# youssefg7/dl-sound-classification

Measured on AMD Instinct MI355X. Metric: training clips/sec (EnvNet-v2, ESC-50 shape), higher is better.
Workload: dtype bf16; 1 GPU; EnvNet-v2 train step (BC-mix, fwd, soft-CE, bwd, clip, Adam), ESC-50 shape; global_batch=256, per_gpu_batch=256, clip_samples=220500, parallelism=dp1, model=envnet_v2

## Files before the change

### dl-sound-classification_amd/csrc/pool.hip

```cpp
#include <cstdlib>

#include "channel_partials.h"

namespace {

constexpr int NT = CP_NT;

struct FastDiv {
  uint32_t d, m, l;
};
static FastDiv make_fastdiv(uint32_t d) {
  uint32_t l = 0;
  while ((1u << l) < d) ++l;
  const uint32_t m = (uint32_t)((((uint64_t)1 << 32) * (((uint64_t)1 << l) - d)) / d + 1);
  return FastDiv{d, m, l};
}
__device__ __forceinline__ uint32_t fdiv(uint32_t n, const FastDiv& f) { return (__umulhi(n, f.m) + n) >> f.l; }

__device__ __forceinline__ int64_t out_index(int layout, int b, int oy, int ox, int c, int OH, int OW, int C) {
  if (layout == 0) return (((int64_t)b * OH + oy) * OW + ox) * C + c;
  if (layout == 1) return ((int64_t)b * C + c) * OW + ox;
  return (((int64_t)b * C + c) * OH + oy) * OW + ox;
}

// ... 354 lines not shown
    }
    store8(dz, dtype, off, g);
  }
  cp_fold<2>(s1, s2, C, G, rslots, blockIdx.x, partial);
}

__global__ __launch_bounds__(NT) void pool_bwd_sparse_kernel(const void* __restrict__ dout, int layout,
                                                             const uint8_t* __restrict__ argmax,
                                                             const void* __restrict__ x,
                                                             const void* __restrict__ win, int dtype, int n, int H,
                                                             int W, int C, int kh, int kw,
                                                             const float* __restrict__ scale,
                                                             const float* __restrict__ shift,
                                                             const float* __restrict__ mean,
                                                             const float* __restrict__ invstd,
                                                             float* __restrict__ gm,
                                                             float* __restrict__ partial) {
  const int OH = H / kh, OW = W / kw, G = C / 8;
  const int t = threadIdx.x;
  const int cg = t % G, rs = t / G, rslots = NT / G;
  float sc[8], sh[8], mu[8], is[8];
#pragma unroll
  for (int i = 0; i < 8; ++i) {
    sc[i] = scale[cg * 8 + i]; sh[i] = shift[cg * 8 + i]; mu[i] = mean[cg * 8 + i]; is[i] = invstd[cg * 8 + i];
  }
  float s1[8] = {0}, s2[8] = {0};
  const int cells = n * OH * OW;
  for (int cell = blockIdx.x * rslots + rs; cell < cells; cell += gridDim.x * rslots) {
    const int ox = cell % OW;
    const int q = cell / OW;
    const int oy = q % OH;
// ... 11 lines not shown
        const uint32_t word = i < 4 ? am.x : am.y;
        const int a = (int)((word >> (8 * (i & 3))) & 0xffu);
        const int iy = oy * kh + a / kw, ix = ox * kw + a % kw;
        xv[i] = ld_elem(x, dtype, (((int64_t)b * H + iy) * W + ix) * C + cg * 8 + i);
        dv[i] = ld_elem(dout, dtype, out_index(layout, b, oy, ox, cg * 8 + i, OH, OW, C));
      }
    }
    float gv[8];
#pragma unroll
    for (int i = 0; i < 8; ++i) {
      const float g = fmaf(xv[i], sc[i], sh[i]) > 0.f ? dv[i] : 0.f;
      gv[i] = g;
      s1[i] += g;
      s2[i] = fmaf(g, (xv[i] - mu[i]) * is[i], s2[i]);
    }
    float4* gq = reinterpret_cast<float4*>(gm + (int64_t)cell * C + cg * 8);
    gq[0] = make_float4(gv[0], gv[1], gv[2], gv[3]);
    gq[1] = make_float4(gv[4], gv[5], gv[6], gv[7]);
  }
  __shared__ float red[NT * 16];
#pragma unroll
  for (int i = 0; i < 8; ++i) { red[t * 16 + i] = s1[i]; red[t * 16 + 8 + i] = s2[i]; }
  __syncthreads();
  for (int e = t; e < 2 * C; e += NT) {
    const int qq = e / C, c = e % C, g2 = c / 8, ci = c % 8;
    float acc = 0.f;
    for (int r2 = 0; r2 < rslots; ++r2) acc += red[(r2 * G + g2) * 16 + qq * 8 + ci];
    partial[((int64_t)blockIdx.x * C + c) * 2 + qq] = acc;
  }
}

__global__ __launch_bounds__(NT) void pool_bwd_sparse_tr_kernel(const void* __restrict__ dout,
                                                                const uint8_t* __restrict__ argmax,
                                                                const void* __restrict__ x,
                                                                const void* __restrict__ win, int dtype, int cells,
                                                                int H, int W, int C, int kh, int kw, int lg_nch,
                                                                const float* __restrict__ scale,
                                                                const float* __restrict__ shift,
                                                                const float* __restrict__ mean,
                                                                const float* __restrict__ invstd,
                                                                float* __restrict__ gm, float* __restrict__ partial) {
  const int OW = W / kw, S = (H / kh) * OW, G = C / 8;
  const int t = threadIdx.x;
  const int lb = xcd_block_id();
  const int cg = t % G, rs = t / G, rslots = NT / G;
  const int LD = C + 4;
  __shared__ __attribute__((aligned(16))) float red[NT * 16];
  float* tile = red;
  float sc[8], sh[8], mu[8], is[8];
#pragma unroll
  for (int i = 0; i < 8; ++i) {
    sc[i] = scale[cg * 8 + i]; sh[i] = shift[cg * 8 + i]; mu[i] = mean[cg * 8 + i]; is[i] = invstd[cg * 8 + i];
  }
  float s1[8] = {0}, s2[8] = {0};
  const int es = dtype == MIA_BF16 ? 1 : 2;
  const uintptr_t dbase = reinterpret_cast<uintptr_t>(dout) >> es;
// ... 51 lines not shown
        for (int i = 0; i < 8; ++i) {
          const uint32_t word = i < 4 ? am.x : am.y;
          const int a = (int)((word >> (8 * (i & 3))) & 0xffu);
          const int iy = oy * kh + a / kw, ix = ox * kw + a % kw;
          xv[i] = ld_elem(x, dtype, (((int64_t)b * H + iy) * W + ix) * C + cg * 8 + i);
        }
      }
      float gv[8];
#pragma unroll
      for (int i = 0; i < 8; ++i) {
        const float g = fmaf(xv[i], sc[i], sh[i]) > 0.f ? dv[i] : 0.f;
        gv[i] = g;
        s1[i] += g;
        s2[i] = fmaf(g, (xv[i] - mu[i]) * is[i], s2[i]);
      }
      float4* gq = reinterpret_cast<float4*>(gm + cell * C + cg * 8);
      gq[0] = make_float4(gv[0], gv[1], gv[2], gv[3]);
      gq[1] = make_float4(gv[4], gv[5], gv[6], gv[7]);
    }
    __syncthreads();
  }
  cp_fold<2>(s1, s2, C, G, rslots, lb, partial, red);
}

__global__ __launch_bounds__(NT) void pool_bn_bwd_apply_oct_kernel(const float* __restrict__ gm,
                                                                   const uint8_t* __restrict__ argmax,
                                                                   const bf16* __restrict__ x, int n, int H, int W,
                                                                   int C, int kh, int kw, FastDiv dNO, FastDiv dH,
                                                                   FastDiv dG, const float* __restrict__ gamma,
                                                                   const float* __restrict__ mean,
                                                                   const float* __restrict__ invstd,
                                                                   const float* __restrict__ dgamma,
                                                                   const float* __restrict__ dbeta, bf16* dx,
                                                                   float* __restrict__ partial) {
  const int OH = H / kh, OW = W / kw, G = C / 8, NO = (W + 7) / 8;
  const int t = threadIdx.x;
  const int cg = t % G;
  const int P = n * H * W;
  float mu[8], is[8], a[8], mb[8], mg[8];
  const float invP = 1.f / (float)P;
// ... 6 lines not shown
    mg[i] = dgamma[c] * invP;
  }
  float s1[8] = {0};
  const int64_t units = (int64_t)n * H * NO * G;
  for (int64_t u = (int64_t)blockIdx.x * NT + t; u < units; u += (int64_t)gridDim.x * NT) {
    const int rest = (int)fdiv((uint32_t)(u), dG);
    const int rowi = (int)fdiv((uint32_t)rest, dNO);
    const int o8 = rest - rowi * NO;
    const int iy = rowi - (int)fdiv((uint32_t)rowi, dH) * H;
    const int b = (rowi - iy) / H;
    const int ix0 = o8 * 8;
    const int oy = iy / kh, ox = ix0 / kw;
    const bool cell = oy < OH && ox < OW;
    const int64_t coff = cell ? (((int64_t)b * OH + oy) * OW + ox) * C + cg * 8 : 0;
    const uint2 am = *reinterpret_cast<const uint2*>(argmax + coff);
    const float4 g0 = reinterpret_cast<const float4*>(gm + coff)[0];
    const float4 g1 = reinterpret_cast<const float4*>(gm + coff)[1];
    const int64_t xoff = ((int64_t)rowi * W + ix0) * C + cg * 8;
    uint4 xr[8];
#pragma unroll
    for (int j = 0; j < 8; ++j) {
      const int64_t o = ix0 + j < W ? xoff + (int64_t)j * C : xoff;
      xr[j] = *reinterpret_cast<const uint4*>(x + o);
    }
    const float gv[8] = {g0.x, g0.y, g0.z, g0.w, g1.x, g1.y, g1.z, g1.w};
    const int pos0 = (iy - oy * kh) * kw + (ix0 - ox * kw);
#pragma unroll
    for (int j = 0; j < 8; ++j) {
      if (ix0 + j >= W) break;
      const uint32_t w4[4] = {xr[j].x, xr[j].y, xr[j].z, xr[j].w};
      uint32_t o4[4];
#pragma unroll
      for (int q = 0; q < 4; ++q) {
        float g[2];
#pragma unroll
        for (int h = 0; h < 2; ++h) {
          const int i = 2 * q + h;
          const float xv = __uint_as_float(h ? (w4[q] & 0xffff0000u) : (w4[q] << 16));
          const uint32_t word = i < 4 ? am.x : am.y;
          const int av = (int)((word >> (8 * (i & 3))) & 0xffu);
          const float gi = cell && av == pos0 + j ? gv[i] : 0.f;
          g[h] = a[i] * (gi - mb[i] - (xv - mu[i]) * is[i] * mg[i]);
          s1[i] += g[h];
        }
        o4[q] = pk_bf16(g[0], g[1]);
      }
      *reinterpret_cast<uint4*>(dx + xoff + (int64_t)j * C) = uint4{o4[0], o4[1], o4[2], o4[3]};
    }
  }
  if (partial) cp_fold<1>(s1, nullptr, C, G, NT / G, blockIdx.x, partial);
}

template <int KW, int RU>
__global__ __launch_bounds__(NT) void pool_bn_bwd_apply_run_kernel(const float* __restrict__ gm,
                                                                   const uint8_t* __restrict__ argmax,
                                                                   const bf16* __restrict__ x, int n, int H, int W,
                                                                   int C, int kh, FastDiv dNR, FastDiv dH, FastDiv dG,
                                                                   const float* __restrict__ gamma,
                                                                   const float* __restrict__ mean,
                                                                   const float* __restrict__ invstd,
                                                                   const float* __restrict__ dgamma,
                                                                   const float* __restrict__ dbeta, bf16* dx,
                                                                   float* __restrict__ partial) {
  const int OH = H / kh, OW = W / KW, G = C / 8, NR = (W + KW - 1) / KW;
  const int t = threadIdx.x;
  const int cg = t % G;
  const int P = n * H * W;
  float mu[8], is[8], a[8], mb[8], mg[8];
  const float invP = 1.f / (float)P;
#pragma unroll
  for (int i = 0; i < 8; ++i) {
    const int c = cg * 8 + i;
    mu[i] = mean[c]; is[i] = invstd[c];
    a[i] = (gamma ? gamma[c] : 1.f) * is[i];
    mb[i] = dbeta[c] * invP;
    mg[i] = dgamma[c] * invP;
  }
  float s1[8] = {0};
  const int units = n * H * NR * G;
  const int stride = gridDim.x * NT;
  for (int u0 = blockIdx.x * NT + t; u0 < units; u0 += RU * stride) {
    uint4 xr[RU][KW];
    uint2 am[RU];
    float4 g0[RU], g1[RU];
    int64_t xoff[RU];
    int pos0[RU], ix0[RU];
#pragma unroll
    for (int v = 0; v < RU; ++v) {
      const int u = min(u0 + v * stride, units - 1);
      const int rest = (int)fdiv((uint32_t)u, dG);
      const int rowi = (int)fdiv((uint32_t)rest, dNR);
      const int run = rest - rowi * NR;
      const int b = (int)fdiv((uint32_t)rowi, dH);
      const int iy = rowi - b * H;
      ix0[v] = run * KW;
      const int oy = iy / kh;
      const bool cell = oy < OH && run < OW;
      const int64_t coff = cell ? (((int64_t)b * OH + oy) * OW + run) * C + cg * 8 : 0;
      pos0[v] = cell ? (iy - oy * kh) * KW : -256;
      am[v] = *reinterpret_cast<const uint2*>(argmax + coff);
      g0[v] = reinterpret_cast<const float4*>(gm + coff)[0];
      g1[v] = reinterpret_cast<const float4*>(gm + coff)[1];
      xoff[v] = ((int64_t)rowi * W + ix0[v]) * C + cg * 8;
#pragma unroll
      for (int j = 0; j < KW; ++j) {
        const int64_t o = ix0[v] + j < W ? xoff[v] + (int64_t)j * C : xoff[v];
        xr[v][j] = *reinterpret_cast<const uint4*>(x + o);
      }
    }
#pragma unroll
    for (int v = 0; v < RU; ++v) {
      if (u0 + v * stride >= units) break;
      const float gv[8] = {g0[v].x, g0[v].y, g0[v].z, g0[v].w, g1[v].x, g1[v].y, g1[v].z, g1[v].w};
#pragma unroll
      for (int j = 0; j < KW; ++j) {
        if (ix0[v] + j >= W) break;
        const uint32_t w4[4] = {xr[v][j].x, xr[v][j].y, xr[v][j].z, xr[v][j].w};
        uint32_t o4[4];
#pragma unroll
        for (int q = 0; q < 4; ++q) {
          float g[2];
#pragma unroll
          for (int h = 0; h < 2; ++h) {
            const int i = 2 * q + h;
            const float xv = __uint_as_float(h ? (w4[q] & 0xffff0000u) : (w4[q] << 16));
            const uint32_t word = i < 4 ? am[v].x : am[v].y;
            const int av = (int)((word >> (8 * (i & 3))) & 0xffu);
            const float gi = av == pos0[v] + j ? gv[i] : 0.f;
// ... 6 lines not shown
      }
    }
  }
  if (partial) cp_fold<1>(s1, nullptr, C, G, NT / G, blockIdx.x, partial);
}

#ifndef PB_UNROLL
#define PB_UNROLL 4
#endif
#ifndef PB_NB
#define PB_NB CP_MAXBLK
#endif
#ifndef PB_RUNS
#define PB_RUNS 1
#endif
__global__ __launch_bounds__(NT) void pool_bn_bwd_apply_kernel(const float* __restrict__ gm,
                                                               const uint8_t* __restrict__ argmax,
                                                               const void* __restrict__ x, int dtype, int n, int H,
                                                               int W, int C, int kh, int kw, FastDiv dW, FastDiv dH,
                                                               FastDiv dkw, FastDiv dkh,
                                                               const float* __restrict__ gamma,
                                                               const float* __restrict__ mean,
                                                               const float* __restrict__ invstd,
                                                               const float* __restrict__ dgamma,
                                                               const float* __restrict__ dbeta, void* dx,
                                                               float* __restrict__ partial) {
  const int OH = H / kh, OW = W / kw, G = C / 8;
  const int t = threadIdx.x;
  const int cg = t % G, rs = t / G, rslots = NT / G;
  const int P = n * H * W;
  float mu[8], is[8], a[8], mb[8], mg[8];
  const float invP = 1.f / (float)P;
#pragma unroll
  for (int i = 0; i < 8; ++i) {
    const int c = cg * 8 + i;
    mu[i] = mean[c]; is[i] = invstd[c];
    a[i] = (gamma ? gamma[c] : 1.f) * is[i];
    mb[i] = dbeta[c] * invP;
    mg[i] = dgamma[c] * invP;
  }
  float s1[8] = {0};
  const int stride = gridDim.x * rslots;
  for (int r0 = blockIdx.x * rslots + rs; r0 < P; r0 += PB_UNROLL * stride) {
    float xv[PB_UNROLL][8];
    uint2 am[PB_UNROLL];
    float4 g0[PB_UNROLL], g1[PB_UNROLL];
#pragma unroll
    for (int u = 0; u < PB_UNROLL; ++u) {
      const int r = min(r0 + u * stride, P - 1);
      load8(x, dtype, (int64_t)r * C + cg * 8, xv[u]);
      const int q = (int)fdiv(r, dW), ix = r - q * W;
      const int b = (int)fdiv(q, dH), iy = q - b * H;
      const int oy = min((int)fdiv(iy, dkh), OH - 1), ox = min((int)fdiv(ix, dkw), OW - 1);
      const int64_t coff = (((int64_t)b * OH + oy) * OW + ox) * C + cg * 8;
      am[u] = *reinterpret_cast<const uint2*>(argmax + coff);
      g0[u] = reinterpret_cast<const float4*>(gm + coff)[0];
      g1[u] = reinterpret_cast<const float4*>(gm + coff)[1];
    }
#pragma unroll
    for (int u = 0; u < PB_UNROLL; ++u) {
      const int r = r0 + u * stride;
      if (r >= P) break;
      const int q = (int)fdiv(r, dW), ix = r - q * W;
      const int iy = q - (int)fdiv(q, dH) * H;
      const int oy = (int)fdiv(iy, dkh), ox = (int)fdiv(ix, dkw);
      const int pos = oy < OH && ox < OW ? (iy - oy * kh) * kw + (ix - ox * kw) : -1;
      const float gv[8] = {g0[u].x, g0[u].y, g0[u].z, g0[u].w, g1[u].x, g1[u].y, g1[u].z, g1[u].w};
      float g[8];
#pragma unroll
      for (int i = 0; i < 8; ++i) {
        const uint32_t word = i < 4 ? am[u].x : am[u].y;
        const int av = (int)((word >> (8 * (i & 3))) & 0xffu);
        const float gi = av == pos ? gv[i] : 0.f;
        g[i] = a[i] * (gi - mb[i] - (xv[u][i] - mu[i]) * is[i] * mg[i]);
        s1[i] += g[i];
      }
      store8(dx, dtype, (int64_t)r * C + cg * 8, g);
    }
  }
  if (partial) cp_fold<1>(s1, nullptr, C, G, rslots, blockIdx.x, partial);
}

// ... 94 lines not shown
  MIA_CHECK_ARG(c % 8 == 0 && c >= 8 && (NT % (c / 8)) == 0, "pool_bwd: channels");
  MIA_CHECK_ARG((int64_t)n * h * w < (1ll << 31), "pool_bwd: too many pixels for 32-bit indexing");
  const int rslots = NT / (c / 8);
  const int64_t P = (int64_t)n * h * w;
  hipStream_t s = as_stream(stream);
  const int nb = (int)std::max<int64_t>(1, std::min<int64_t>(cdiv(P, (int64_t)rslots * 8), CP_MAXBLK));
  pool_bwd_kernel<<<nb, NT, 0, s>>>(dout, out_layout, argmax, x, dtype, n, h, w, c, kh, kw, scale, shift, mean,
                                    invstd, dz, (float*)partial);
  MIA_LAUNCH_CHECK("pool_bwd");
  cp_final2_kernel<<<(unsigned)c, 256, 0, s>>>((const float*)partial, nb, c,  dbeta,
                                                dgamma);
  MIA_LAUNCH_CHECK("pool_bwd_final");
  return 0;
}

extern "C" int mia_pool_bwd_gather(const void* dout, int32_t out_layout, const uint8_t* argmax, const void* x,
                                   const void* win, int32_t dtype, int32_t n, int32_t h, int32_t w, int32_t c, int32_t kh, int32_t kw,
                                   const float* scale, const float* shift, const float* mean, const float* invstd,
                                   float* gm, float* dgamma, float* dbeta, void* partial, mia_stream_t stream) {
  MIA_CHECK_ARG(dout && argmax && x && scale && shift && mean && invstd && gm && dgamma && dbeta && partial,
                "pool_bwd_gather: null pointer");
  MIA_CHECK_ARG(c % 8 == 0 && c >= 8 && (NT % (c / 8)) == 0, "pool_bwd_gather: channels");
  MIA_CHECK_ARG((int64_t)n * h * w < (1ll << 31), "pool_bwd_gather: too many pixels for 32-bit indexing");
  MIA_CHECK_ARG(h >= kh && w >= kw && kh * kw <= 256 && (reinterpret_cast<uintptr_t>(gm) & 15) == 0,
                "pool_bwd_gather: bad geometry / alignment");
  const int rslots = NT / (c / 8);
  const int64_t cells = (int64_t)n * (h / kh) * (w / kw);
  const int nb = (int)std::max<int64_t>(1, std::min<int64_t>(cdiv(cells, (int64_t)rslots * 2), CP_MAXBLK));
  hipStream_t s = as_stream(stream);
  MIA_CHECK_ARG(!win || (reinterpret_cast<uintptr_t>(win) & 15) == 0, "pool_bwd_gather: win alignment");
  if (!pool_v1() && (out_layout == 2 || (out_layout == 1 && h / kh == 1)) && rslots >= 16 &&
      cells < (1ll << 31) - 1024) {
    int lg_nch = 0;
    while ((4 << lg_nch) < rslots) ++lg_nch;
    pool_bwd_sparse_tr_kernel<<<nb, NT, 0, s>>>(dout, argmax, x, win, dtype, (int)cells, h, w, c, kh, kw, lg_nch, scale,
                                                shift, mean, invstd, gm, (float*)partial);
  } else {
    pool_bwd_sparse_kernel<<<nb, NT, 0, s>>>(dout, out_layout, argmax, x, win, dtype, n, h, w, c, kh, kw, scale, shift,
                                             mean, invstd, gm, (float*)partial);
  }
  MIA_LAUNCH_CHECK("pool_bwd_gather");
  cp_final2_kernel<<<(unsigned)c, 256, 0, s>>>((const float*)partial, nb, c,  dbeta,
                                                dgamma);
  MIA_LAUNCH_CHECK("pool_bwd_gather_final");
  return 0;
}

extern "C" int mia_pool_bn_relu_bwd_apply(const float* gm, const uint8_t* argmax, const void* x, int32_t dtype,
                                          int32_t n, int32_t h, int32_t w, int32_t c, int32_t kh, int32_t kw,
                                          const float* gamma, const float* mean, const float* invstd,
                                          const float* dgamma, const float* dbeta, void* dx, float* dbias,
                                          void* partial, mia_stream_t stream) {
  MIA_CHECK_ARG(gm && argmax && x && mean && invstd && dgamma && dbeta && dx, "pool_bn_bwd_apply: null pointer");
  MIA_CHECK_ARG(!dbias || partial, "pool_bn_bwd_apply: dbias needs the partial workspace");
  MIA_CHECK_ARG(c % 8 == 0 && c >= 8 && (NT % (c / 8)) == 0, "pool_bn_bwd_apply: channels");
  MIA_CHECK_ARG((int64_t)n * h * w < (1ll << 31), "pool_bn_bwd_apply: too many pixels for 32-bit indexing");
  MIA_CHECK_ARG(h >= kh && w >= kw && kh * kw <= 256, "pool_bn_bwd_apply: bad geometry");
  const int rslots = NT / (c / 8);
  const int64_t P = (int64_t)n * h * w;
  hipStream_t s = as_stream(stream);
  const int64_t units = (int64_t)n * h * ((w + 7) / 8) * (c / 8);
  if (kw % 8 == 0 && dtype == MIA_BF16 && units < (1ll << 31) &&
      ((reinterpret_cast<uintptr_t>(x) | reinterpret_cast<uintptr_t>(dx)) & 15) == 0) {
    const int nb = (int)std::max<int64_t>(1, std::min<int64_t>(cdiv(units, NT), CP_MAXBLK));
    pool_bn_bwd_apply_oct_kernel<<<nb, NT, 0, s>>>(gm, argmax, reinterpret_cast<const bf16*>(x), n, h, w, c, kh, kw,
                                                   make_fastdiv((w + 7) / 8), make_fastdiv(h), make_fastdiv(c / 8),
                                                   gamma, mean, invstd, dgamma, dbeta, reinterpret_cast<bf16*>(dx),
                                                   dbias ? (float*)partial : nullptr);
    MIA_LAUNCH_CHECK("pool_bn_bwd_apply");
    if (dbias) {
      cp_final2_kernel<<<(unsigned)c, 256, 0, s>>>((const float*)partial, nb, c,  dbias, nullptr);
      MIA_LAUNCH_CHECK("pool_bn_bwd_apply_final");
    }
    return 0;
  }
  const int64_t runs = (int64_t)n * h * cdiv(w, kw) * (c / 8);
  static const bool per_pixel = getenv("MIA_POOL_BWD_PIXEL") != nullptr;
  if (kw >= 2 && kw <= 4 && dtype == MIA_BF16 && runs < (1ll << 31) && !per_pixel &&
      ((reinterpret_cast<uintptr_t>(x) | reinterpret_cast<uintptr_t>(dx)) & 15) == 0) {
    constexpr int RU = PB_RUNS;
    const int nb = (int)std::max<int64_t>(1, std::min<int64_t>(cdiv(runs, (int64_t)NT * RU), PB_NB));
    const FastDiv dNR = make_fastdiv((int)cdiv(w, kw)), dH = make_fastdiv(h), dG = make_fastdiv(c / 8);
    float* part = dbias ? (float*)partial : nullptr;
    const bf16* xb = reinterpret_cast<const bf16*>(x);
    bf16* dxb = reinterpret_cast<bf16*>(dx);
    if (kw == 2)
      pool_bn_bwd_apply_run_kernel<2, RU><<<nb, NT, 0, s>>>(gm, argmax, xb, n, h, w, c, kh, dNR, dH, dG, gamma, mean,
                                                            invstd, dgamma, dbeta, dxb, part);
    else if (kw == 3)
      pool_bn_bwd_apply_run_kernel<3, RU><<<nb, NT, 0, s>>>(gm, argmax, xb, n, h, w, c, kh, dNR, dH, dG, gamma, mean,
                                                            invstd, dgamma, dbeta, dxb, part);
    else
      pool_bn_bwd_apply_run_kernel<4, RU><<<nb, NT, 0, s>>>(gm, argmax, xb, n, h, w, c, kh, dNR, dH, dG, gamma, mean,
                                                            invstd, dgamma, dbeta, dxb, part);
    MIA_LAUNCH_CHECK("pool_bn_bwd_apply_run");
    if (dbias) {
      cp_final2_kernel<<<(unsigned)c, 256, 0, s>>>((const float*)partial, nb, c,  dbias, nullptr);
      MIA_LAUNCH_CHECK("pool_bn_bwd_apply_final");
    }
    return 0;
  }
  const int nb = (int)std::max<int64_t>(1, std::min<int64_t>(cdiv(P, (int64_t)rslots * 8), CP_MAXBLK));
  pool_bn_bwd_apply_kernel<<<nb, NT, 0, s>>>(gm, argmax, x, dtype, n, h, w, c, kh, kw, make_fastdiv(w), make_fastdiv(h),
                                             make_fastdiv(kw), make_fastdiv(kh), gamma, mean, invstd, dgamma,
                                             dbeta, dx, dbias ? (float*)partial : nullptr);
  MIA_LAUNCH_CHECK("pool_bn_bwd_apply");
  if (dbias) {
    cp_final2_kernel<<<(unsigned)c, 256, 0, s>>>((const float*)partial, nb, c,  dbias, nullptr);
    MIA_LAUNCH_CHECK("pool_bn_bwd_apply_final");
  }
  return 0;
}

extern "C" int mia_col2im_rows(const float* p, int32_t n, int32_t ph, int32_t w, int32_t kh, void* out, int32_t dtype,
                               mia_stream_t stream) {
  MIA_CHECK_ARG(p && out && n > 0 && ph > 0 && w > 0 && kh > 0, "col2im_rows: bad arguments");
  MIA_CHECK_ARG((int64_t)n * (ph + kh - 1) * w < (1ll << 31), "col2im_rows: too many elements");
  const int64_t total = (int64_t)n * (ph + kh - 1) * w;
  const int nb = (int)std::min<int64_t>(cdiv(total, 256), 16384);
  col2im_rows_kernel<<<nb, 256, 0, as_stream(stream)>>>(p, n, ph, w, kh, out, dtype);
  MIA_LAUNCH_CHECK("col2im_rows");
  return 0;
}
```

### dl-sound-classification_amd/src/miaudio/kernels.py

```python
from __future__ import annotations

import math
from dataclasses import dataclass

import os

import torch

from . import lib as L

_WS: dict = {}


def workspace(nbytes: int, device, slot: str = "main") -> torch.Tensor:
    key = (str(device), slot)
    buf = _WS.get(key)
    nbytes = max(int(nbytes), 256)
    if buf is None or buf.numel() < nbytes:
        buf = torch.empty(int(nbytes * 1.25) + 256, dtype=torch.uint8, device=device)
        _WS[key] = buf
    return buf


def _s():
# ... 285 lines not shown
    ws = workspace(lib.mia_bn_partial_bytes(P, C), x.device, "bn")
    L.check(lib.mia_bn_bwd_apply(dz.data_ptr(), x.data_ptr(), dx.data_ptr(), L.dtype_code(x), P, C,
                                 L.ptr(gamma), bn.mean.data_ptr(), bn.invstd.data_ptr(), dgamma.data_ptr(),
                                 dbeta.data_ptr(), L.ptr(dbias), ws.data_ptr(), _s()), "mia_bn_bwd_apply")


def bn_relu_bwd_apply(dact, x, dx, P, C, gamma, bn: BNState, dgamma, dbeta, dbias=None):
    lib = L.load()
    ws = workspace(lib.mia_bn_partial_bytes(P, C), x.device, "bn")
    L.check(lib.mia_bn_relu_bwd_apply(dact.data_ptr(), x.data_ptr(), dx.data_ptr(), L.dtype_code(x), P, C,
                                      L.ptr(gamma), bn.scale.data_ptr(), bn.shift.data_ptr(), bn.mean.data_ptr(),
                                      bn.invstd.data_ptr(), dgamma.data_ptr(), dbeta.data_ptr(), L.ptr(dbias),
                                      ws.data_ptr(), _s()), "mia_bn_relu_bwd_apply")


def pool_bwd_gather(dout, out_layout, argmax, x, n, h, w, c, kh, kw, bn: BNState, win=None):
    if win is not None and (win.dtype != x.dtype or win.numel() != n * (h // kh) * (w // kw) * c):
        raise ValueError("pool_bwd_gather: win must hold one x-typed value per pooled cell and channel")
    dev = x.device
    g = torch.empty(2, c, dtype=torch.float32, device=dev)
    gm = torch.empty(n * (h // kh) * (w // kw), c, dtype=torch.float32, device=dev)
    lib = L.load()
    ws = workspace(lib.mia_bn_partial_bytes(n * h * w, c), dev, "bn")
    L.check(lib.mia_pool_bwd_gather(dout.data_ptr(), out_layout, argmax.data_ptr(), x.data_ptr(), L.ptr(win),
                                    L.dtype_code(x), n, h, w, c, kh, kw, bn.scale.data_ptr(), bn.shift.data_ptr(), bn.mean.data_ptr(),
                                    bn.invstd.data_ptr(), gm.data_ptr(), g[0].data_ptr(), g[1].data_ptr(),
                                    ws.data_ptr(), _s()), "mia_pool_bwd_gather")
    return gm, g[0], g[1]


def pool_bn_relu_bwd_apply(gm, argmax, x, n, h, w, c, kh, kw, gamma, bn: BNState, dgamma, dbeta, dx, dbias=None):
    lib = L.load()
    ws = workspace(lib.mia_bn_partial_bytes(n * h * w, c), x.device, "bn")
    L.check(lib.mia_pool_bn_relu_bwd_apply(gm.data_ptr(), argmax.data_ptr(), x.data_ptr(), L.dtype_code(x), n, h, w,
                                           c, kh, kw, L.ptr(gamma), bn.mean.data_ptr(), bn.invstd.data_ptr(),
                                           dgamma.data_ptr(), dbeta.data_ptr(), dx.data_ptr(), L.ptr(dbias),
                                           ws.data_ptr(), _s()), "mia_pool_bn_relu_bwd_apply")


def pool_fwd(x, n, h, w, c, kh, kw, bn: BNState, out, out_layout, argmax, win=None):
    if win is not None and (win.dtype != x.dtype or win.numel() != n * (h // kh) * (w // kw) * c):
        raise ValueError("pool_fwd: win must hold one x-typed value per pooled cell and channel")
    L.check(L.load().mia_pool_fwd(x.data_ptr(), L.dtype_code(x), n, h, w, c, kh, kw, bn.scale.data_ptr(),
                                  bn.shift.data_ptr(), out.data_ptr(), out_layout, argmax.data_ptr(), L.ptr(win),
                                  _s()),
            "mia_pool_fwd")


def pool_raw_stats(x, n, h, w, c, kh, kw, gamma, kshift, win, argmax):
    assert x.dtype == torch.bfloat16 and win.dtype == torch.bfloat16 and x.is_contiguous()
    nblk = 2048
    part = torch.empty(nblk, c, 2, dtype=torch.float32, device=x.device)
# ... 759 lines not shown
```

### dl-sound-classification_amd/src/miaudio/lib.py

```python
from __future__ import annotations

import ctypes as C
import os
from pathlib import Path

import torch

PKG_ROOT = Path(__file__).resolve().parents[2]
LIB_PATH = Path(os.environ.get("MIAUDIO_LIB") or PKG_ROOT / "lib" / "libmiaudio.so")

F32, BF16, U8 = 0, 1, 2
MXFP8 = 16
OP_DENSE, OP_CONV, OP_CONVROW = 0, 1, 2
KC, RC = 0, 1
PRE_NONE, PRE_AFFINE, PRE_AFFINE_RELU, PRE_GELU = 0, 1, 2, 3
ACT_NONE, ACT_RELU, ACT_GELU, DACT_NZ, DACT_GELU, ACT_ADD_AUX, ACT_GELU_SAVE = 0, 1, 2, 3, 4, 5, 6
ACT_GELU_SAVE_D, DACT_MUL = 7, 8

vp = C.c_void_p
i32 = C.c_int32
i64 = C.c_int64
f32 = C.c_float


# ... 55 lines not shown
    "mia_gemm_mxfp8_ex": (C.c_int, [vp, vp, i64, vp, vp, i64, P(MiaEpilogue), i64, i64, i64, vp, vp]),
    "mia_layernorm_fwd_mx": (C.c_int, [vp, i32, vp, vp, vp, vp, vp, vp, vp, i64, i32, f32, vp]),
    "mia_attn_fwd_mx": (C.c_int, [vp, vp, vp, vp, vp, i32, i32, i32, f32, vp]),
    "mia_splitk_reduce": (C.c_int, [vp, i32, i64, i64, P(MiaEpilogue), vp]),
    "mia_logmel_workspace_bytes": (i64, [i64, i64]),
    "mia_logmel_fwd": (C.c_int, [vp, i64, i64, i64, P(MiaMelCfg), vp, vp, vp, vp, vp, vp, vp, vp, vp, vp, vp]),
    "mia_bn_partial_bytes": (i64, [i64, i32]),
    "mia_bn_fwd_stats": (C.c_int, [vp, i32, i64, i32, vp, vp, vp, vp, f32, f32, i32, vp, vp, vp, vp, vp, vp]),
    "mia_bn_relu_bwd_reduce": (C.c_int, [vp, vp, vp, i32, i64, i32, vp, vp, vp, vp, vp, vp, vp, vp]),
    "mia_bn_bwd_apply": (C.c_int, [vp, vp, vp, i32, i64, i32, vp, vp, vp, vp, vp, vp, vp, vp]),
    "mia_bn_relu_bwd_apply": (C.c_int, [vp, vp, vp, i32, i64, i32, vp, vp, vp, vp, vp, vp, vp, vp, vp, vp]),
    "mia_pool_bwd_gather": (C.c_int, [vp, i32, vp, vp, vp, i32, i32, i32, i32, i32, i32, i32, vp, vp, vp, vp, vp, vp,
                                      vp, vp, vp]),
    "mia_pool_bn_relu_bwd_apply": (C.c_int, [vp, vp, vp, i32, i32, i32, i32, i32, i32, i32, vp, vp, vp, vp, vp, vp,
                                             vp, vp, vp]),
    "mia_pool_fwd": (C.c_int, [vp, i32, i32, i32, i32, i32, i32, i32, vp, vp, vp, i32, vp, vp, vp]),
    "mia_pool_bwd_bn_relu_reduce": (C.c_int, [vp, i32, vp, vp, i32, i32, i32, i32, i32, i32, i32, vp, vp, vp,
                                              vp, vp, vp, vp, vp, vp]),
    "mia_colsum": (C.c_int, [vp, i32, i64, i32, i64, vp, vp, vp]),
    "mia_col2im_rows": (C.c_int, [vp, i32, i32, i32, i32, vp, i32, vp]),
    "mia_conv1ch_dgrad": (C.c_int, [vp, vp, vp, i32, i32, i32, vp]),
    "mia_fe_conv2_fwd": (C.c_int, [vp, vp, vp, vp, vp, vp, i32, i32, i32, vp]),
    "mia_fe_conv2_dgrad": (C.c_int, [vp, vp, vp, i32, i32, i32, vp]),
    "mia_bn_relu_apply": (C.c_int, [vp, i64, i32, vp, vp, vp, vp]),
    "mia_shift_pad_w2": (C.c_int, [vp, i64, i32, i32, vp, vp]),
    "mia_pad_w2": (C.c_int, [vp, i64, i32, i32, vp, vp, i32, vp]),
    "mia_drop_last_col": (C.c_int, [vp, i64, i32, i32, vp, vp]),
    "mia_fe_conv1_fwd": (C.c_int, [vp, vp, vp, vp, vp, i32, i32, i32, vp]),
    "mia_fe_conv3_fwd": (C.c_int, [vp, vp, vp, vp, vp, i32, i32, i32, i32, vp]),
    "mia_pool_raw_stats": (C.c_int, [vp, i32, i32, i32, i32, i32, i32, vp, vp, vp, vp, vp, i32, vp]),
# ... 152 lines not shown
```

Baseline: 15780 clips/s.

## Store pool backward gradient buffer in bf16 and add raw-window gather kernel

The intermediate pooled gradient buffer gm, passed between the pool backward gather and the BN-ReLU backward apply, now defaults to the activation dtype (bf16) instead of f32. This halves its write and read traffic. A new gather kernel for the row-major layout with a saved window reads win and dout as packed vectors directly, instead of decoding argmax and doing per-element gathers from x. The cost is extra gradient rounding to bf16 in the intermediate, which an env var can override back to f32.

```diff
diff --git a/dl-sound-classification_amd/csrc/pool.hip b/dl-sound-classification_amd/csrc/pool.hip
--- a/dl-sound-classification_amd/csrc/pool.hip
+++ b/dl-sound-classification_amd/csrc/pool.hip
@@ -1,5 +1,6 @@
 #include <cstdlib>
 
+#include "../../include/miaudio_pool.h"
 #include "channel_partials.h"
 
 namespace {
@@ -392,7 +393,7 @@
                                                              const float* __restrict__ shift,
                                                              const float* __restrict__ mean,
                                                              const float* __restrict__ invstd,
-                                                             float* __restrict__ gm,
+                                                             void* __restrict__ gm, int gdt,
                                                              float* __restrict__ partial) {
   const int OH = H / kh, OW = W / kw, G = C / 8;
   const int t = threadIdx.x;
@@ -434,9 +435,7 @@
       s1[i] += g;
       s2[i] = fmaf(g, (xv[i] - mu[i]) * is[i], s2[i]);
     }
-    float4* gq = reinterpret_cast<float4*>(gm + (int64_t)cell * C + cg * 8);
-    gq[0] = make_float4(gv[0], gv[1], gv[2], gv[3]);
-    gq[1] = make_float4(gv[4], gv[5], gv[6], gv[7]);
+    store8(gm, gdt, (int64_t)cell * C + cg * 8, gv);
   }
   __shared__ float red[NT * 16];
 #pragma unroll
@@ -448,6 +447,75 @@
     for (int r2 = 0; r2 < rslots; ++r2) acc += red[(r2 * G + g2) * 16 + qq * 8 + ci];
     partial[((int64_t)blockIdx.x * C + c) * 2 + qq] = acc;
   }
+}
+
+template <int DT>
+struct Raw8 {
+  uint4 v[DT == MIA_BF16 ? 1 : 2];
+  __device__ __forceinline__ void load(const void* p, int64_t off) {
+    const uint4* q = reinterpret_cast<const uint4*>(reinterpret_cast<const char*>(p) + off * (DT == MIA_BF16 ? 2 : 4));
+    v[0] = q[0];
+    if constexpr (DT != MIA_BF16) v[1] = q[1];
+  }
+  __device__ __forceinline__ void unpack(float (&f)[8]) const {
+    if constexpr (DT == MIA_BF16) {
+      const uint32_t w[4] = {v[0].x, v[0].y, v[0].z, v[0].w};
+#pragma unroll
+      for (int i = 0; i < 4; ++i) { f[2 * i] = __uint_as_float(w[i] << 16); f[2 * i + 1] = __uint_as_float(w[i] & 0xffff0000u); }
+    } else {
+      const uint32_t w[8] = {v[0].x, v[0].y, v[0].z, v[0].w, v[1].x, v[1].y, v[1].z, v[1].w};
+#pragma unroll
+      for (int i = 0; i < 8; ++i) f[i] = __uint_as_float(w[i]);
+    }
+  }
+};
+
+#ifndef PG_DEPTH
+#define PG_DEPTH 1
+#endif
+template <int DT, int GDT, int D>
+__global__ __launch_bounds__(NT) void pool_bwd_sparse_ra_kernel(const void* __restrict__ dout,
+                                                                const void* __restrict__ win, int cells, int C,
+                                                                const float* __restrict__ scale,
+                                                                const float* __restrict__ shift,
+                                                                const float* __restrict__ mean,
+                                                                const float* __restrict__ invstd,
+                                                                void* __restrict__ gm, float* __restrict__ partial) {
+  const int G = C / 8;
+  const int t = threadIdx.x;
+  const int cg = t % G, rs = t / G, rslots = NT / G;
+  float sc[8], sh[8], mu[8], is[8];
+#pragma unroll
+  for (int i = 0; i < 8; ++i) {
+    sc[i] = scale[cg * 8 + i]; sh[i] = shift[cg * 8 + i]; mu[i] = mean[cg * 8 + i]; is[i] = invstd[cg * 8 + i];
+  }
+  float s1[8] = {0}, s2[8] = {0};
+  const int stride = gridDim.x * rslots;
+  for (int cell0 = blockIdx.x * rslots + rs; cell0 < cells; cell0 += D * stride) {
+    Raw8<DT> wr[D], dr[D];
+#pragma unroll
+    for (int v = 0; v < D; ++v) {
+      const int64_t off = (int64_t)min(cell0 + v * stride, cells - 1) * C + cg * 8;
+      wr[v].load(win, off);
+      dr[v].load(dout, off);
+    }
+#pragma unroll
+    for (int v = 0; v < D; ++v) {
+      const bool live = cell0 + v * stride < cells;
+      float xv[8], dv[8], gv[8];
+      wr[v].unpack(xv);
+      dr[v].unpack(dv);
+#pragma unroll
+      for (int i = 0; i < 8; ++i) {
+        const float g = fmaf(xv[i], sc[i], sh[i]) > 0.f ? dv[i] : 0.f;
+        gv[i] = g;
+        s1[i] = live ? s1[i] + g : s1[i];
+        s2[i] = live ? fmaf(g, (xv[i] - mu[i]) * is[i], s2[i]) : s2[i];
+      }
+      if (live) store8(gm, GDT, (int64_t)(cell0 + v * stride) * C + cg * 8, gv);
+    }
+  }
+  cp_fold<2>(s1, s2, C, G, rslots, blockIdx.x, partial);
 }
 
 __global__ __launch_bounds__(NT) void pool_bwd_sparse_tr_kernel(const void* __restrict__ dout,
@@ -459,7 +527,8 @@
                                                                 const float* __restrict__ shift,
                                                                 const float* __restrict__ mean,
                                                                 const float* __restrict__ invstd,
-                                                                float* __restrict__ gm, float* __restrict__ partial) {
+                                                                void* __restrict__ gm, int gdt,
+                                                                float* __restrict__ partial) {
   const int OW = W / kw, S = (H / kh) * OW, G = C / 8;
   const int t = threadIdx.x;
   const int lb = xcd_block_id();
@@ -541,16 +610,15 @@
         s1[i] += g;
         s2[i] = fmaf(g, (xv[i] - mu[i]) * is[i], s2[i]);
       }
-      float4* gq = reinterpret_cast<float4*>(gm + cell * C + cg * 8);
-      gq[0] = make_float4(gv[0], gv[1], gv[2], gv[3]);
-      gq[1] = make_float4(gv[4], gv[5], gv[6], gv[7]);
+      store8(gm, gdt, cell * C + cg * 8, gv);
     }
     __syncthreads();
   }
   cp_fold<2>(s1, s2, C, G, rslots, lb, partial, red);
 }
 
-__global__ __launch_bounds__(NT) void pool_bn_bwd_apply_oct_kernel(const float* __restrict__ gm,
+template <int GDT>
+__global__ __launch_bounds__(NT) void pool_bn_bwd_apply_oct_kernel(const void* __restrict__ gm,
                                                                    const uint8_t* __restrict__ argmax,
                                                                    const bf16* __restrict__ x, int n, int H, int W,
                                                                    int C, int kh, int kw, FastDiv dNO, FastDiv dH,
@@ -587,8 +655,8 @@
     const bool cell = oy < OH && ox < OW;
     const int64_t coff = cell ? (((int64_t)b * OH + oy) * OW + ox) * C + cg * 8 : 0;
     const uint2 am = *reinterpret_cast<const uint2*>(argmax + coff);
-    const float4 g0 = reinterpret_cast<const float4*>(gm + coff)[0];
-    const float4 g1 = reinterpret_cast<const float4*>(gm + coff)[1];
+    Raw8<GDT> gr;
+    gr.load(gm, coff);
     const int64_t xoff = ((int64_t)rowi * W + ix0) * C + cg * 8;
     uint4 xr[8];
 #pragma unroll
@@ -596,7 +664,8 @@
       const int64_t o = ix0 + j < W ? xoff + (int64_t)j * C : xoff;
       xr[j] = *reinterpret_cast<const uint4*>(x + o);
     }
-    const float gv[8] = {g0.x, g0.y, g0.z, g0.w, g1.x, g1.y, g1.z, g1.w};
+    float gv[8];
+    gr.unpack(gv);
     const int pos0 = (iy - oy * kh) * kw + (ix0 - ox * kw);
 #pragma unroll
     for (int j = 0; j < 8; ++j) {
@@ -624,8 +693,8 @@
   if (partial) cp_fold<1>(s1, nullptr, C, G, NT / G, blockIdx.x, partial);
 }
 
-template <int KW, int RU>
-__global__ __launch_bounds__(NT) void pool_bn_bwd_apply_run_kernel(const float* __restrict__ gm,
+template <int KW, int RU, int GDT>
+__global__ __launch_bounds__(NT) void pool_bn_bwd_apply_run_kernel(const void* __restrict__ gm,
                                                                    const uint8_t* __restrict__ argmax,
                                                                    const bf16* __restrict__ x, int n, int H, int W,
                                                                    int C, int kh, FastDiv dNR, FastDiv dH, FastDiv dG,
@@ -655,7 +724,7 @@
   for (int u0 = blockIdx.x * NT + t; u0 < units; u0 += RU * stride) {
     uint4 xr[RU][KW];
     uint2 am[RU];
-    float4 g0[RU], g1[RU];
+    Raw8<GDT> gr[RU];
     int64_t xoff[RU];
     int pos0[RU], ix0[RU];
 #pragma unroll
@@ -672,8 +741,7 @@
       const int64_t coff = cell ? (((int64_t)b * OH + oy) * OW + run) * C + cg * 8 : 0;
       pos0[v] = cell ? (iy - oy * kh) * KW : -256;
       am[v] = *reinterpret_cast<const uint2*>(argmax + coff);
-      g0[v] = reinterpret_cast<const float4*>(gm + coff)[0];
-      g1[v] = reinterpret_cast<const float4*>(gm + coff)[1];
+      gr[v].load(gm, coff);
       xoff[v] = ((int64_t)rowi * W + ix0[v]) * C + cg * 8;
 #pragma unroll
       for (int j = 0; j < KW; ++j) {
@@ -684,7 +752,8 @@
 #pragma unroll
     for (int v = 0; v < RU; ++v) {
       if (u0 + v * stride >= units) break;
-      const float gv[8] = {g0[v].x, g0[v].y, g0[v].z, g0[v].w, g1[v].x, g1[v].y, g1[v].z, g1[v].w};
+      float gv[8];
+      gr[v].unpack(gv);
 #pragma unroll
       for (int j = 0; j < KW; ++j) {
         if (ix0[v] + j >= W) break;
@@ -721,7 +790,8 @@
 #ifndef PB_RUNS
 #define PB_RUNS 1
 #endif
-__global__ __launch_bounds__(NT) void pool_bn_bwd_apply_kernel(const float* __restrict__ gm,
+template <int GDT>
+__global__ __launch_bounds__(NT) void pool_bn_bwd_apply_kernel(const void* __restrict__ gm,
                                                                const uint8_t* __restrict__ argmax,
                                                                const void* __restrict__ x, int dtype, int n, int H,
                                                                int W, int C, int kh, int kw, FastDiv dW, FastDiv dH,
@@ -751,7 +821,7 @@
   for (int r0 = blockIdx.x * rslots + rs; r0 < P; r0 += PB_UNROLL * stride) {
     float xv[PB_UNROLL][8];
     uint2 am[PB_UNROLL];
-    float4 g0[PB_UNROLL], g1[PB_UNROLL];
+    Raw8<GDT> gr[PB_UNROLL];
 #pragma unroll
     for (int u = 0; u < PB_UNROLL; ++u) {
       const int r = min(r0 + u * stride, P - 1);
@@ -761,8 +831,7 @@
       const int oy = min((int)fdiv(iy, dkh), OH - 1), ox = min((int)fdiv(ix, dkw), OW - 1);
       const int64_t coff = (((int64_t)b * OH + oy) * OW + ox) * C + cg * 8;
       am[u] = *reinterpret_cast<const uint2*>(argmax + coff);
-      g0[u] = reinterpret_cast<const float4*>(gm + coff)[0];
-      g1[u] = reinterpret_cast<const float4*>(gm + coff)[1];
+      gr[u].load(gm, coff);
     }
 #pragma unroll
     for (int u = 0; u < PB_UNROLL; ++u) {
@@ -772,7 +841,8 @@
       const int iy = q - (int)fdiv(q, dH) * H;
       const int oy = (int)fdiv(iy, dkh), ox = (int)fdiv(ix, dkw);
       const int pos = oy < OH && ox < OW ? (iy - oy * kh) * kw + (ix - ox * kw) : -1;
-      const float gv[8] = {g0[u].x, g0[u].y, g0[u].z, g0[u].w, g1[u].x, g1[u].y, g1[u].z, g1[u].w};
+      float gv[8];
+      gr[u].unpack(gv);
       float g[8];
 #pragma unroll
       for (int i = 0; i < 8; ++i) {
@@ -897,30 +967,53 @@
   return 0;
 }
 
-extern "C" int mia_pool_bwd_gather(const void* dout, int32_t out_layout, const uint8_t* argmax, const void* x,
-                                   const void* win, int32_t dtype, int32_t n, int32_t h, int32_t w, int32_t c, int32_t kh, int32_t kw,
-                                   const float* scale, const float* shift, const float* mean, const float* invstd,
-                                   float* gm, float* dgamma, float* dbeta, void* partial, mia_stream_t stream) {
+static int pool_grid_cap(int nb) {
+  const char* e = getenv("MIA_POOL_GRID");
+  const int cap = e ? atoi(e) : 0;
+  return cap > 0 ? std::min(nb, cap) : nb;
+}
+
+extern "C" int mia_pool_bwd_gather_ex(const void* dout, int32_t out_layout, const uint8_t* argmax, const void* x,
+                                      const void* win, int32_t dtype, int32_t n, int32_t h, int32_t w, int32_t c,
+                                      int32_t kh, int32_t kw, const float* scale, const float* shift,
+                                      const float* mean, const float* invstd, void* gm, int32_t gm_dtype,
+                                      float* dgamma, float* dbeta, void* partial, mia_stream_t stream) {
   MIA_CHECK_ARG(dout && argmax && x && scale && shift && mean && invstd && gm && dgamma && dbeta && partial,
                 "pool_bwd_gather: null pointer");
   MIA_CHECK_ARG(c % 8 == 0 && c >= 8 && (NT % (c / 8)) == 0, "pool_bwd_gather: channels");
   MIA_CHECK_ARG((int64_t)n * h * w < (1ll << 31), "pool_bwd_gather: too many pixels for 32-bit indexing");
   MIA_CHECK_ARG(h >= kh && w >= kw && kh * kw <= 256 && (reinterpret_cast<uintptr_t>(gm) & 15) == 0,
                 "pool_bwd_gather: bad geometry / alignment");
+  MIA_CHECK_ARG(gm_dtype == MIA_F32 || (gm_dtype == MIA_BF16 && dtype == MIA_BF16),
+                "pool_bwd_gather: gm is f32, or bf16 beside bf16 activations (gm dtype %d, dtype %d)", gm_dtype, dtype);
   const int rslots = NT / (c / 8);
   const int64_t cells = (int64_t)n * (h / kh) * (w / kw);
-  const int nb = (int)std::max<int64_t>(1, std::min<int64_t>(cdiv(cells, (int64_t)rslots * 2), CP_MAXBLK));
+  const int nb = pool_grid_cap((int)std::max<int64_t>(1, std::min<int64_t>(cdiv(cells, (int64_t)rslots * 2), CP_MAXBLK)));
   hipStream_t s = as_stream(stream);
   MIA_CHECK_ARG(!win || (reinterpret_cast<uintptr_t>(win) & 15) == 0, "pool_bwd_gather: win alignment");
-  if (!pool_v1() && (out_layout == 2 || (out_layout == 1 && h / kh == 1)) && rslots >= 16 &&
-      cells < (1ll << 31) - 1024) {
+  const bool v1 = pool_v1();
+  const bool chmajor = out_layout == 2 || (out_layout == 1 && h / kh == 1);
+  if (!v1 && chmajor && rslots >= 16 && cells < (1ll << 31) - 1024) {
     int lg_nch = 0;
     while ((4 << lg_nch) < rslots) ++lg_nch;
     pool_bwd_sparse_tr_kernel<<<nb, NT, 0, s>>>(dout, argmax, x, win, dtype, (int)cells, h, w, c, kh, kw, lg_nch, scale,
-                                                shift, mean, invstd, gm, (float*)partial);
+                                                shift, mean, invstd, gm, gm_dtype, (float*)partial);
+  } else if (!v1 && win && out_layout == 0 && (dtype == MIA_BF16 || dtype == MIA_F32) &&
+             (reinterpret_cast<uintptr_t>(dout) & 15) == 0 && cells + (int64_t)PG_DEPTH * nb * rslots < (1ll << 31)) {
+    float* part = (float*)partial;
+    const int nc = (int)cells;
+    if (dtype == MIA_F32)
+      pool_bwd_sparse_ra_kernel<MIA_F32, MIA_F32, PG_DEPTH><<<nb, NT, 0, s>>>(dout, win, nc, c, scale, shift, mean,
+                                                                              invstd, gm, part);
+    else if (gm_dtype == MIA_F32)
+      pool_bwd_sparse_ra_kernel<MIA_BF16, MIA_F32, PG_DEPTH><<<nb, NT, 0, s>>>(dout, win, nc, c, scale, shift, mean,
+                                                                               invstd, gm, part);
+    else
+      pool_bwd_sparse_ra_kernel<MIA_BF16, MIA_BF16, PG_DEPTH><<<nb, NT, 0, s>>>(dout, win, nc, c, scale, shift, mean,
+                                                                                invstd, gm, part);
   } else {
     pool_bwd_sparse_kernel<<<nb, NT, 0, s>>>(dout, out_layout, argmax, x, win, dtype, n, h, w, c, kh, kw, scale, shift,
-                                             mean, invstd, gm, (float*)partial);
+                                             mean, invstd, gm, gm_dtype, (float*)partial);
   }
   MIA_LAUNCH_CHECK("pool_bwd_gather");
   cp_final2_kernel<<<(unsigned)c, 256, 0, s>>>((const float*)partial, nb, c,  dbeta,
@@ -929,27 +1022,29 @@
   return 0;
 }
 
-extern "C" int mia_pool_bn_relu_bwd_apply(const float* gm, const uint8_t* argmax, const void* x, int32_t dtype,
-                                          int32_t n, int32_t h, int32_t w, int32_t c, int32_t kh, int32_t kw,
-                                          const float* gamma, const float* mean, const float* invstd,
-                                          const float* dgamma, const float* dbeta, void* dx, float* dbias,
-                                          void* partial, mia_stream_t stream) {
-  MIA_CHECK_ARG(gm && argmax && x && mean && invstd && dgamma && dbeta && dx, "pool_bn_bwd_apply: null pointer");
-  MIA_CHECK_ARG(!dbias || partial, "pool_bn_bwd_apply: dbias needs the partial workspace");
-  MIA_CHECK_ARG(c % 8 == 0 && c >= 8 && (NT % (c / 8)) == 0, "pool_bn_bwd_apply: channels");
-  MIA_CHECK_ARG((int64_t)n * h * w < (1ll << 31), "pool_bn_bwd_apply: too many pixels for 32-bit indexing");
-  MIA_CHECK_ARG(h >= kh && w >= kw && kh * kw <= 256, "pool_bn_bwd_apply: bad geometry");
+extern "C" int mia_pool_bwd_gather(const void* dout, int32_t out_layout, const uint8_t* argmax, const void* x,
+                                   const void* win, int32_t dtype, int32_t n, int32_t h, int32_t w, int32_t c, int32_t kh, int32_t kw,
+                                   const float* scale, const float* shift, const float* mean, const float* invstd,
+                                   float* gm, float* dgamma, float* dbeta, void* partial, mia_stream_t stream) {
+  return mia_pool_bwd_gather_ex(dout, out_layout, argmax, x, win, dtype, n, h, w, c, kh, kw, scale, shift, mean, invstd,
+                                gm, MIA_F32, dgamma, dbeta, partial, stream);
+}
+
+template <int GDT>
+static int pool_bn_bwd_apply_launch(const void* gm, const uint8_t* argmax, const void* x, int32_t dtype, int32_t n,
+                                    int32_t h, int32_t w, int32_t c, int32_t kh, int32_t kw, const float* gamma,
+                                    const float* mean, const float* invstd, const float* dgamma, const float* dbeta,
+                                    void* dx, float* dbias, void* partial, hipStream_t s) {
   const int rslots = NT / (c / 8);
   const int64_t P = (int64_t)n * h * w;
-  hipStream_t s = as_stream(stream);
   const int64_t units = (int64_t)n * h * ((w + 7) / 8) * (c / 8);
   if (kw % 8 == 0 && dtype == MIA_BF16 && units < (1ll << 31) &&
       ((reinterpret_cast<uintptr_t>(x) | reinterpret_cast<uintptr_t>(dx)) & 15) == 0) {
     const int nb = (int)std::max<int64_t>(1, std::min<int64_t>(cdiv(units, NT), CP_MAXBLK));
-    pool_bn_bwd_apply_oct_kernel<<<nb, NT, 0, s>>>(gm, argmax, reinterpret_cast<const bf16*>(x), n, h, w, c, kh, kw,
-                                                   make_fastdiv((w + 7) / 8), make_fastdiv(h), make_fastdiv(c / 8),
-                                                   gamma, mean, invstd, dgamma, dbeta, reinterpret_cast<bf16*>(dx),
-                                                   dbias ? (float*)partial : nullptr);
+    pool_bn_bwd_apply_oct_kernel<GDT><<<nb, NT, 0, s>>>(gm, argmax, reinterpret_cast<const bf16*>(x), n, h, w, c, kh, kw,
+                                                        make_fastdiv((w + 7) / 8), make_fastdiv(h), make_fastdiv(c / 8),
+                                                        gamma, mean, invstd, dgamma, dbeta, reinterpret_cast<bf16*>(dx),
+                                                        dbias ? (float*)partial : nullptr);
     MIA_LAUNCH_CHECK("pool_bn_bwd_apply");
     if (dbias) {
       cp_final2_kernel<<<(unsigned)c, 256, 0, s>>>((const float*)partial, nb, c,  dbias, nullptr);
@@ -968,14 +1063,14 @@
     const bf16* xb = reinterpret_cast<const bf16*>(x);
     bf16* dxb = reinterpret_cast<bf16*>(dx);
     if (kw == 2)
-      pool_bn_bwd_apply_run_kernel<2, RU><<<nb, NT, 0, s>>>(gm, argmax, xb, n, h, w, c, kh, dNR, dH, dG, gamma, mean,
-                                                            invstd, dgamma, dbeta, dxb, part);
+      pool_bn_bwd_apply_run_kernel<2, RU, GDT><<<nb, NT, 0, s>>>(gm, argmax, xb, n, h, w, c, kh, dNR, dH, dG, gamma,
+                                                                 mean, invstd, dgamma, dbeta, dxb, part);
     else if (kw == 3)
-      pool_bn_bwd_apply_run_kernel<3, RU><<<nb, NT, 0, s>>>(gm, argmax, xb, n, h, w, c, kh, dNR, dH, dG, gamma, mean,
-                                                            invstd, dgamma, dbeta, dxb, part);
+      pool_bn_bwd_apply_run_kernel<3, RU, GDT><<<nb, NT, 0, s>>>(gm, argmax, xb, n, h, w, c, kh, dNR, dH, dG, gamma,
+                                                                 mean, invstd, dgamma, dbeta, dxb, part);
     else
-      pool_bn_bwd_apply_run_kernel<4, RU><<<nb, NT, 0, s>>>(gm, argmax, xb, n, h, w, c, kh, dNR, dH, dG, gamma, mean,
-                                                            invstd, dgamma, dbeta, dxb, part);
+      pool_bn_bwd_apply_run_kernel<4, RU, GDT><<<nb, NT, 0, s>>>(gm, argmax, xb, n, h, w, c, kh, dNR, dH, dG, gamma,
+                                                                 mean, invstd, dgamma, dbeta, dxb, part);
     MIA_LAUNCH_CHECK("pool_bn_bwd_apply_run");
     if (dbias) {
       cp_final2_kernel<<<(unsigned)c, 256, 0, s>>>((const float*)partial, nb, c,  dbias, nullptr);
@@ -984,15 +1079,44 @@
     return 0;
   }
   const int nb = (int)std::max<int64_t>(1, std::min<int64_t>(cdiv(P, (int64_t)rslots * 8), CP_MAXBLK));
-  pool_bn_bwd_apply_kernel<<<nb, NT, 0, s>>>(gm, argmax, x, dtype, n, h, w, c, kh, kw, make_fastdiv(w), make_fastdiv(h),
-                                             make_fastdiv(kw), make_fastdiv(kh), gamma, mean, invstd, dgamma,
-                                             dbeta, dx, dbias ? (float*)partial : nullptr);
+  pool_bn_bwd_apply_kernel<GDT><<<nb, NT, 0, s>>>(gm, argmax, x, dtype, n, h, w, c, kh, kw, make_fastdiv(w),
+                                                  make_fastdiv(h), make_fastdiv(kw), make_fastdiv(kh), gamma, mean,
+                                                  invstd, dgamma, dbeta, dx, dbias ? (float*)partial : nullptr);
   MIA_LAUNCH_CHECK("pool_bn_bwd_apply");
   if (dbias) {
     cp_final2_kernel<<<(unsigned)c, 256, 0, s>>>((const float*)partial, nb, c,  dbias, nullptr);
     MIA_LAUNCH_CHECK("pool_bn_bwd_apply_final");
   }
   return 0;
+}
+
+extern "C" int mia_pool_bn_relu_bwd_apply_ex(const void* gm, int32_t gm_dtype, const uint8_t* argmax, const void* x,
+                                             int32_t dtype, int32_t n, int32_t h, int32_t w, int32_t c, int32_t kh,
+                                             int32_t kw, const float* gamma, const float* mean, const float* invstd,
+                                             const float* dgamma, const float* dbeta, void* dx, float* dbias,
+                                             void* partial, mia_stream_t stream) {
+  MIA_CHECK_ARG(gm && argmax && x && mean && invstd && dgamma && dbeta && dx, "pool_bn_bwd_apply: null pointer");
+  MIA_CHECK_ARG(!dbias || partial, "pool_bn_bwd_apply: dbias needs the partial workspace");
+  MIA_CHECK_ARG(c % 8 == 0 && c >= 8 && (NT % (c / 8)) == 0, "pool_bn_bwd_apply: channels");
+  MIA_CHECK_ARG((int64_t)n * h * w < (1ll << 31), "pool_bn_bwd_apply: too many pixels for 32-bit indexing");
+  MIA_CHECK_ARG(h >= kh && w >= kw && kh * kw <= 256, "pool_bn_bwd_apply: bad geometry");
+  MIA_CHECK_ARG(gm_dtype == MIA_F32 || gm_dtype == MIA_BF16, "pool_bn_bwd_apply: gm dtype %d", gm_dtype);
+  MIA_CHECK_ARG((reinterpret_cast<uintptr_t>(gm) & 15) == 0, "pool_bn_bwd_apply: gm alignment");
+  hipStream_t s = as_stream(stream);
+  if (gm_dtype == MIA_BF16)
+    return pool_bn_bwd_apply_launch<MIA_BF16>(gm, argmax, x, dtype, n, h, w, c, kh, kw, gamma, mean, invstd, dgamma,
+                                              dbeta, dx, dbias, partial, s);
+  return pool_bn_bwd_apply_launch<MIA_F32>(gm, argmax, x, dtype, n, h, w, c, kh, kw, gamma, mean, invstd, dgamma, dbeta,
+                                           dx, dbias, partial, s);
+}
+
+extern "C" int mia_pool_bn_relu_bwd_apply(const float* gm, const uint8_t* argmax, const void* x, int32_t dtype,
+                                          int32_t n, int32_t h, int32_t w, int32_t c, int32_t kh, int32_t kw,
+                                          const float* gamma, const float* mean, const float* invstd,
+                                          const float* dgamma, const float* dbeta, void* dx, float* dbias,
+                                          void* partial, mia_stream_t stream) {
+  return mia_pool_bn_relu_bwd_apply_ex(gm, MIA_F32, argmax, x, dtype, n, h, w, c, kh, kw, gamma, mean, invstd, dgamma,
+                                       dbeta, dx, dbias, partial, stream);
 }
 
 extern "C" int mia_col2im_rows(const float* p, int32_t n, int32_t ph, int32_t w, int32_t kh, void* out, int32_t dtype,
diff --git a/dl-sound-classification_amd/src/miaudio/kernels.py b/dl-sound-classification_amd/src/miaudio/kernels.py
--- a/dl-sound-classification_amd/src/miaudio/kernels.py
+++ b/dl-sound-classification_amd/src/miaudio/kernels.py
@@ -323,28 +323,32 @@
                                       ws.data_ptr(), _s()), "mia_bn_relu_bwd_apply")
 
 
-def pool_bwd_gather(dout, out_layout, argmax, x, n, h, w, c, kh, kw, bn: BNState, win=None):
+def pool_bwd_gather(dout, out_layout, argmax, x, n, h, w, c, kh, kw, bn: BNState, win=None, gm_dtype=None):
     if win is not None and (win.dtype != x.dtype or win.numel() != n * (h // kh) * (w // kw) * c):
         raise ValueError("pool_bwd_gather: win must hold one x-typed value per pooled cell and channel")
+    if gm_dtype is None:
+        gm_dtype = torch.float32 if os.environ.get("MIA_POOL_GM32", "")[:1] == "1" else x.dtype
     dev = x.device
     g = torch.empty(2, c, dtype=torch.float32, device=dev)
-    gm = torch.empty(n * (h // kh) * (w // kw), c, dtype=torch.float32, device=dev)
+    gm = torch.empty(n * (h // kh) * (w // kw), c, dtype=gm_dtype, device=dev)
     lib = L.load()
     ws = workspace(lib.mia_bn_partial_bytes(n * h * w, c), dev, "bn")
-    L.check(lib.mia_pool_bwd_gather(dout.data_ptr(), out_layout, argmax.data_ptr(), x.data_ptr(), L.ptr(win),
-                                    L.dtype_code(x), n, h, w, c, kh, kw, bn.scale.data_ptr(), bn.shift.data_ptr(), bn.mean.data_ptr(),
-                                    bn.invstd.data_ptr(), gm.data_ptr(), g[0].data_ptr(), g[1].data_ptr(),
-                                    ws.data_ptr(), _s()), "mia_pool_bwd_gather")
+    L.check(lib.mia_pool_bwd_gather_ex(dout.data_ptr(), out_layout, argmax.data_ptr(), x.data_ptr(), L.ptr(win),
+                                       L.dtype_code(x), n, h, w, c, kh, kw, bn.scale.data_ptr(), bn.shift.data_ptr(),
+                                       bn.mean.data_ptr(), bn.invstd.data_ptr(), gm.data_ptr(), L.dtype_code(gm),
+                                       g[0].data_ptr(), g[1].data_ptr(), ws.data_ptr(), _s()),
+            "mia_pool_bwd_gather_ex")
     return gm, g[0], g[1]
 
 
 def pool_bn_relu_bwd_apply(gm, argmax, x, n, h, w, c, kh, kw, gamma, bn: BNState, dgamma, dbeta, dx, dbias=None):
     lib = L.load()
     ws = workspace(lib.mia_bn_partial_bytes(n * h * w, c), x.device, "bn")
-    L.check(lib.mia_pool_bn_relu_bwd_apply(gm.data_ptr(), argmax.data_ptr(), x.data_ptr(), L.dtype_code(x), n, h, w,
-                                           c, kh, kw, L.ptr(gamma), bn.mean.data_ptr(), bn.invstd.data_ptr(),
-                                           dgamma.data_ptr(), dbeta.data_ptr(), dx.data_ptr(), L.ptr(dbias),
-                                           ws.data_ptr(), _s()), "mia_pool_bn_relu_bwd_apply")
+    L.check(lib.mia_pool_bn_relu_bwd_apply_ex(gm.data_ptr(), L.dtype_code(gm), argmax.data_ptr(), x.data_ptr(),
+                                              L.dtype_code(x), n, h, w, c, kh, kw, L.ptr(gamma), bn.mean.data_ptr(),
+                                              bn.invstd.data_ptr(), dgamma.data_ptr(), dbeta.data_ptr(),
+                                              dx.data_ptr(), L.ptr(dbias), ws.data_ptr(), _s()),
+            "mia_pool_bn_relu_bwd_apply_ex")
 
 
 def pool_fwd(x, n, h, w, c, kh, kw, bn: BNState, out, out_layout, argmax, win=None):
diff --git a/dl-sound-classification_amd/src/miaudio/lib.py b/dl-sound-classification_amd/src/miaudio/lib.py
--- a/dl-sound-classification_amd/src/miaudio/lib.py
+++ b/dl-sound-classification_amd/src/miaudio/lib.py
@@ -93,6 +93,10 @@
                                       vp, vp, vp]),
     "mia_pool_bn_relu_bwd_apply": (C.c_int, [vp, vp, vp, i32, i32, i32, i32, i32, i32, i32, vp, vp, vp, vp, vp, vp,
                                              vp, vp, vp]),
+    "mia_pool_bwd_gather_ex": (C.c_int, [vp, i32, vp, vp, vp, i32, i32, i32, i32, i32, i32, i32, vp, vp, vp, vp, vp,
+                                         i32, vp, vp, vp, vp]),
+    "mia_pool_bn_relu_bwd_apply_ex": (C.c_int, [vp, i32, vp, vp, i32, i32, i32, i32, i32, i32, i32, vp, vp, vp, vp, vp,
+                                                vp, vp, vp, vp]),
     "mia_pool_fwd": (C.c_int, [vp, i32, i32, i32, i32, i32, i32, i32, vp, vp, vp, i32, vp, vp, vp]),
     "mia_pool_bwd_bn_relu_reduce": (C.c_int, [vp, i32, vp, vp, i32, i32, i32, i32, i32, i32, i32, vp, vp, vp,
                                               vp, vp, vp, vp, vp, vp]),
diff --git a/include/miaudio_pool.h b/include/miaudio_pool.h
--- /dev/null
+++ b/include/miaudio_pool.h
@@ -0,0 +1,24 @@
+#ifndef MIAUDIO_POOL_H
+#define MIAUDIO_POOL_H
+#include "miaudio.h"
+
+#ifdef __cplusplus
+extern "C" {
+#endif
+
+int mia_pool_bwd_gather_ex(const void* dout, int32_t out_layout, const uint8_t* argmax, const void* x,
+                           const void* win ,
+                           int32_t dtype, int32_t n, int32_t h, int32_t w, int32_t c, int32_t kh, int32_t kw,
+                           const float* scale, const float* shift, const float* mean, const float* invstd,
+                           void* gm, int32_t gm_dtype, float* dgamma, float* dbeta, void* partial,
+                           mia_stream_t stream);
+
+int mia_pool_bn_relu_bwd_apply_ex(const void* gm, int32_t gm_dtype, const uint8_t* argmax, const void* x,
+                                  int32_t dtype, int32_t n, int32_t h, int32_t w, int32_t c, int32_t kh, int32_t kw,
+                                  const float* gamma, const float* mean, const float* invstd, const float* dgamma,
+                                  const float* dbeta, void* dx, float* dbias, void* partial, mia_stream_t stream);
+
+#ifdef __cplusplus
+}
+#endif
+#endif
```

Result: faster. 16000 clips/s, median of 6 (+1.4%).
